# enac-drones/dronesim

Measured on AMD Instinct MI355X. Metric: drone-steps/sec (num_drones x env steps/s), higher is better.
Workload: dtype f32

## Files before the change

dronesim_amd/csrc/dsim_step.hip:

```cpp
#include "dsim_kernels.h"

template <bool NOISE, bool NT, bool EXT, bool CH = false, int SUB = 0, bool ACT = false, bool TC = false, bool MD = false>
__global__ __launch_bounds__(256, EXT ? 3 : DSIM_STEP_WAVES) void k_step_fast(StepK a) {
  static_assert(!MD || (SUB == 1 && !EXT && !ACT && !CH && TC), "MD: the plain single-sub-step TC instances");
  const DevType& T = a.types[0];
  const long long sfs = a.st.field_stride, tfs = a.tg.field_stride;
  const unsigned sl = 4u * kv_lane(a.st, threadIdx.x), tl = 4u * kv_lane(a.tg, threadIdx.x);
  const long long i0 = (long long)blockIdx.x * 256;
  float* const sb = a.st.base + kv_off(a.st, i0);
  const unsigned bt = a.tgt_tiles == ~0u ? (blockIdx.x & a.tgt_mask) : blockIdx.x % a.tgt_tiles;
  const long long i0t = (!EXT && !ACT) ? (long long)bt * 256 : i0;
  const float* const tb = a.tg.base + kv_off(a.tg, i0t);
  Rigid s;
  CtrlMem<4> m;
  Target tg;
  constexpr bool TAB = NOISE && (EXT || SUB != 1);
  __shared__ NoiseTab ntab_[TAB ? 1 : 0 + 1];
  const NoiseTab* const ntab = TAB ? &ntab_[0] : nullptr;
  if (TAB) noise_tab_init(ntab_[0], threadIdx.x);
  load_rigid<NT>(sb, sfs, sl, s);
  load_mem<4, NT, CH || MD>(sb, sfs, sl, m);
  if (TAB) __syncthreads();
  if (CH || MD) { m.last_vel = s.vel; m.last_rates = MD ? body_rates_apart(s.q, s.w) : body_rates(s.q, s.w); }
  const long long i = i0 + threadIdx.x;
  if (NOISE && a.step_index_dev) a.step_index += *a.step_index_dev;
  V3 pos_e;
  float yaw_e;
  if (!EXT) {
    load_target<NT, TC>(tb, tfs, tl, a.tc, tg);
    if (ACT) {
      float act[4];
#pragma unroll
      for (int j = 0; j < 4; ++j) act[j] = clampf(a.action[(long long)j * a.n_pad + i], T.pmin[j], T.pmax[j]);
      quad_substeps<NOISE ? 1 : 0, 4, false, SUB, false, -1, SUB == 0, TAB ? 1 : 0>(T, a, i, s, act, a.step_index, V3{-0.0f, -0.0f, -0.0f}, nullptr, -1, ntab);
    } else {
      quad_substeps<NOISE ? 1 : 0, 4, false, SUB, false, -1, SUB == 0, TAB ? 1 : 0>(T, a, i, s, m.cmd, a.step_index, V3{-0.0f, -0.0f, -0.0f}, nullptr, -1, ntab);
    }
    if (SUB == 1) ground_watch(T, s, a.fb.counters, i < a.n);
    indi_quad<false>(T, a.dt_ctrl, s, tg, m, pos_e, yaw_e);
  } else {
    int wp = 0;
    if (a.wp_table) wp = a.wp_counter[i]; else load_target<NT>(tb, tfs, tl, tg);
    for (int k = 0; k < a.n_steps; ++k) {
      if (a.wp_table) waypoint_target(a, i, wp, tg);
      if (a.substeps > 1) quad_substeps<NOISE ? 1 : 0, 4, false, 0, false, -1, true, TAB ? 1 : 0>(T, a, i, s, m.cmd, a.step_index + k, V3{-0.0f, -0.0f, -0.0f}, nullptr, -1, ntab);
      else quad_substeps<NOISE ? 1 : 0, 4, false, 0, false, -1, false, TAB ? 1 : 0>(T, a, i, s, m.cmd, a.step_index + k, V3{-0.0f, -0.0f, -0.0f}, nullptr, -1, ntab);
      ground_watch(T, s, a.fb.counters, i < a.n);
      indi_quad<false>(T, a.dt_ctrl, s, tg, m, pos_e, yaw_e);
      wp = waypoint_next(wp, a.n_wp);
    }
    if (a.wp_table) a.wp_counter[i] = wp;
  }
  const unsigned so = pin_lane_offset(sl);
  store_rigid<NT>(sb, sfs, so, s);
  store_mem<4, NT, CH>(sb, sfs, so, m);
  if (!EXT && SUB != 1) ground_watch(T, s, a.fb.counters, i < a.n);
}

template <bool NOISE, bool NT, bool S1, bool ACT = false, bool MD = false>
__global__ __launch_bounds__(256, (MD && !NOISE) ? 7 : DSIM_HEXA_WAVES) void k_step_hexa(StepK a) {
  static_assert(!MD || (S1 && !ACT), "MD: the single-sub-step instances without an explicit action");
  const DevType& T = a.types[0];
  const long long sfs = a.st.field_stride, tfs = a.tg.field_stride;
  const unsigned sl = 4u * kv_lane(a.st, threadIdx.x), tl = 4u * kv_lane(a.tg, threadIdx.x);
  const long long i0 = (long long)blockIdx.x * 256;
  float* const sb = a.st.base + kv_off(a.st, i0);
  const float* const tb = a.tg.base + kv_off(a.tg, i0);
  constexpr bool TAB = NOISE && !S1;
  __shared__ NoiseTab ntab_[TAB ? 1 : 0 + 1];
  const NoiseTab* const ntab = TAB ? &ntab_[0] : nullptr;
  if (TAB) noise_tab_init(ntab_[0], threadIdx.x);
  Rigid s;
  CtrlMem<6> m;
  Target tg;
  load_rigid<NT>(sb, sfs, sl, s);
  load_mem<6, NT, MD>(sb, sfs, sl, m);
  load_target<NT>(tb, tfs, tl, tg);
  if (MD) { m.last_vel = s.vel; m.last_rates = body_rates_apart(s.q, s.w); }
  if (TAB) __syncthreads();
  const long long i = i0 + threadIdx.x;
  if (NOISE && a.step_index_dev) a.step_index += *a.step_index_dev;
  V3 pos_e;
  float yaw_e;
  if (ACT) {
    float act[6];
#pragma unroll
    for (int j = 0; j < 6; ++j) act[j] = clampf(a.action[(long long)j * a.n_pad + i], T.pmin[j], T.pmax[j]);
    hexa_substeps<NOISE, false, S1, false, !S1, TAB ? 1 : 0>(T, a, i, s, act, a.step_index, V3{-0.0f, -0.0f, -0.0f}, -1, ntab);
  } else {
    hexa_substeps<NOISE, false, S1, false, !S1, TAB ? 1 : 0>(T, a, i, s, m.cmd, a.step_index, V3{-0.0f, -0.0f, -0.0f}, -1, ntab);
  }
  indi_hexa<false>(T, a.dt_ctrl, s, tg, m, pos_e, yaw_e, a.fb, i);
  float* const sb2 = (DSIM_LATE_STORE_BASE && (!S1 || DSIM_LATE_STORE_BASE_S1)) ? const_cast<float*>(opaque_after(sb, s.pos.x)) : sb;
  const unsigned so = pin_lane_offset(sl);
  store_rigid<NT>(sb2, sfs, so, s);
  store_mem<6, NT>(sb2, sfs, so, m);
  ground_watch(T, s, a.fb.counters, i < a.n);
}

struct MatK { KView st; long long n_pad; };
__global__ __launch_bounds__(256) void k_materialize(MatK a) {
  const long long i = (long long)blockIdx.x * 256 + threadIdx.x;
  if (i >= a.n_pad) return;
  float* p = a.st.base + kv_off(a.st, i);
  const long long fs = a.st.field_stride;
  Rigid s;
  load_rigid(p, fs, 0u, s);
  const V3 wb = body_rates(s.q, s.w);
  p[13 * fs] = s.vel.x; p[14 * fs] = s.vel.y; p[15 * fs] = s.vel.z;
  p[16 * fs] = wb.x; p[17 * fs] = wb.y; p[18 * fs] = wb.z;
}

template <int KIND, bool NOISE, bool NT, bool S1, bool ACT = false>
__device__ __forceinline__ void run_body(const StepK& a, long long i0, long long lo, long long last, int run_type,
                                         const NoiseTab* tab = nullptr) {
  constexpr bool HEXA = KIND != DSIM_DEV_KIND_QUAD;
  const long long i = i0 + threadIdx.x;
  if (i >= last || i < lo) return;
  const DevType& T = a.types[run_type];
  const long long sfs = a.st.field_stride, tfs = a.tg.field_stride;
  const unsigned sl = 4u * kv_lane(a.st, threadIdx.x), tl = 4u * kv_lane(a.tg, threadIdx.x);
  float* const sb = a.st.base + kv_off(a.st, i0);
  const float* const tb = a.tg.base + kv_off(a.tg, i0);
  constexpr int NA = HEXA ? 6 : 4;
  Rigid s;
  CtrlMem<NA> m;
  Target tg;
  load_rigid<NT>(sb, sfs, sl, s);
  load_mem<NA, NT>(sb, sfs, sl, m);
  load_target<NT>(tb, tfs, tl, tg);
  V3 ext = v3(0, 0, 0);
  if (a.ext_force) ext = v3(a.ext_force[i], a.ext_force[a.n_pad + i], a.ext_force[2 * a.n_pad + i]);
  unsigned long long step_index = a.step_index;
  if (NOISE && a.step_index_dev) step_index += *a.step_index_dev;
  V3 pos_e;
  float yaw_e;
  const long long nid = NOISE ? noise_id(a, i) : -1LL;
  float act[NA];
#pragma unroll
  for (int j = 0; j < NA; ++j) act[j] = ACT ? clampf(a.action[(long long)j * a.n_pad + i], T.pmin[j], T.pmax[j]) : m.cmd[j];
  if constexpr (HEXA) {
    hexa_substeps<NOISE, false, S1, false, !S1, (NOISE && !S1 && !ACT) ? 1 : 0>(T, a, i, s, act, step_index, ext, nid, tab);
    if constexpr (KIND == DSIM_DEV_KIND_HEXA) indi_hexa<false>(T, a.dt_ctrl, s, tg, m, pos_e, yaw_e, a.fb, i);
    else indi_quad<false, 6>(T, a.dt_ctrl, s, tg, m, pos_e, yaw_e);
  } else {
    quad_substeps<NOISE ? 1 : 0, 4, false, S1 ? 1 : 0, false, -1, !S1, (NOISE && !S1 && !ACT) ? 1 : 0>(T, a, i, s, act, step_index, ext, nullptr, nid, tab);
    indi_quad<false>(T, a.dt_ctrl, s, tg, m, pos_e, yaw_e);
  }
  const unsigned so = pin_lane_offset(sl);
  float* const sb2 = (DSIM_LATE_STORE_BASE && !S1) ? const_cast<float*>(opaque_after(sb, s.pos.x)) : sb;
  store_rigid<NT>(sb2, sfs, so, s);
  store_mem<NA, NT>(sb2, sfs, so, m);
  ground_watch(T, s, a.fb.counters, i < a.n);
  if (a.bin.count && i < a.n) bin_entry<KIND != DSIM_DEV_KIND_HEXA_QUADLAW>(a.bin, s.pos.x, s.pos.y, s.pos.z, a.bin.local_offset + i);
}
template <int KIND, bool NOISE, bool NT, bool S1>
__global__ __launch_bounds__(256, KIND ? DSIM_HEXA_WAVES : DSIM_STEP_WAVES) void k_step_run(StepK a) {
  DSIM_NOISE_TAB(NOISE && !S1, 256);
  run_body<KIND, NOISE, NT, S1>(a, a.first + (long long)blockIdx.x * 256, a.lo, a.last, a.run_type, ntab);
}
template <bool NOISE, bool NT, bool S1, bool ACT>
__global__ __launch_bounds__(256, 3) void k_step_runs(StepK a, RunTab rt) {
  DSIM_RUN_OF_BLOCK(rt, ro, blockIdx.x);
  DSIM_NOISE_TAB(NOISE && !S1 && !ACT, 256);
  if (ro.hexa) run_body<DSIM_DEV_KIND_HEXA, NOISE, NT, S1, ACT>(a, ro.i0, ro.lo, ro.last, ro.type, ntab);
  else run_body<DSIM_DEV_KIND_QUAD, NOISE, NT, S1, ACT>(a, ro.i0, ro.lo, ro.last, ro.type, ntab);
}

static int step_dyn(dsim_ctx* ctx, const dsim_step_args* args, const StepK& a, hipStream_t st_) {
  const int rc = dyn_check(ctx, args, a);
  if (rc) return rc;
  if (!a.tg.base) return DSIM_E_ARG;
  ctx->prebin.valid = false;
  return dyn_launch(true, a, stream_policy(args, a.n_pad, 256.0), st_);
}

static int step_runs(dsim_ctx* ctx, int64_t n, const dsim_step_args* args, const StepCall& c, StepK& a,
                     const dsim_type_run* runs, int n_runs, hipStream_t st_) {
  const dim3 b(256);
  const bool nt = stream_policy(args, a.n_pad, 240.0);
  bool any_hexa = false;
  bin_next_prepare(ctx, n, args, &a, st_);
  for (int r = 0; r < n_runs; ++r) {
    if (!run_valid(ctx, a.n_pad, runs[r])) return DSIM_E_ARG;
    any_hexa |= ctx->h_types[runs[r].type].kind == DSIM_KIND_HEXA6DOF;
  }
  if (any_hexa) {
    const int rc = fb_open_queue(ctx, &a, st_);
    if (rc) return rc;
  }
  const bool per_run_pays = a.substeps > 1 && a.n_pad >= (1LL << 20) && !args->action;
  const bool one_launch = !c.any_quadlaw6 && !per_run_pays;
  if (n_runs <= DSIM_MAX_TYPES && (n_runs >= 2 || args->action) && one_launch) {
    RunTab rt;
    const int blocks = make_runtab(ctx, a.n_pad, runs, n_runs, &rt, &any_hexa);
    if (blocks < 0) return blocks;
    if (blocks > 0) {
      const dim3 g((unsigned)blocks);
      with_flags([&](auto N, auto NT, auto S1, auto ACT) {
        hipLaunchKernelGGL((k_step_runs<N(), NT() && !ACT(), S1(), ACT()>), g, b, 0, st_, a, rt);
      }, c.noise, nt, a.substeps == 1, args->action != nullptr);
    }
  } else {
    for (int r = 0; r < n_runs; ++r) {
      const dsim_type_run& run = runs[r];
      if (run.count == 0) continue;
      a.first = run.first & ~255LL; a.lo = run.first; a.last = run.first + run.count; a.run_type = run.type;
      const dim3 g(grid_for(a.last - a.first));
      const int kind = ctx->h_types[run.type].kind;
      with_flags([&](auto N, auto NT, auto S1) {
        if (kind == DSIM_KIND_HEXA6DOF) hipLaunchKernelGGL((k_step_run<DSIM_DEV_KIND_HEXA, N(), NT(), S1()>), g, b, 0, st_, a);
        else if (kind == DSIM_KIND_HEXA_QUADLAW) hipLaunchKernelGGL((k_step_run<DSIM_DEV_KIND_HEXA_QUADLAW, N(), false, S1()>), g, b, 0, st_, a);
        else hipLaunchKernelGGL((k_step_run<DSIM_DEV_KIND_QUAD, N(), NT(), S1()>), g, b, 0, st_, a);
      }, c.noise, nt, a.substeps == 1);
    }
  }
  if (any_hexa) fb_finish(ctx, a, st_);
  bin_next_commit(ctx, n, args, a);
  return (int)hipGetLastError();
}

static long long step_quad_tiles(const dsim_step_args* args, const StepCall& c, const StepK& a, hipStream_t st_) {
  const bool nt = stream_policy(args, a.n_pad, 232.0);
  const long long tiles = a.n_pad / 256;
  if (tiles == 0) return 0;
  const dim3 g((unsigned)tiles), b(256);
  const bool ext = c.multi;
  const bool ch = (args->options & DSIM_OPT_CHAINED) != 0;
  const bool tc = tgt_const_honoured(args);
  const bool md = (args->options & DSIM_OPT_MEM_DERIVED) != 0;
  with_flags([&](auto N, auto NT, auto CH, auto S1, auto TC, auto MD) {
    if (ext) hipLaunchKernelGGL((k_step_fast<N(), NT(), true, CH()>), g, b, 0, st_, a);
    else if (args->action) hipLaunchKernelGGL((k_step_fast<N(), false, false, false, S1() ? 1 : 0, true>), g, b, 0, st_, a);
    else hipLaunchKernelGGL((k_step_fast<N(), NT(), false, CH(), S1() ? 1 : 0, false, TC(), MD() && S1() && !CH() && TC()>), g, b, 0, st_, a);
  }, c.noise, nt, ch, a.substeps == 1, tc, md);
  return tiles * 256;
}

static int step_hexa_tiles(dsim_ctx* ctx, const dsim_step_args* args, const StepCall& c, StepK& a, hipStream_t st_, long long* first) {
  const long long tiles = a.n_pad / 256;
  const bool nt = stream_policy(args, a.n_pad, 248.0);
  const int rc = fb_open_queue(ctx, &a, st_);
  if (rc) return rc;
  const dim3 g((unsigned)tiles), b(256);
  const bool md = (args->options & DSIM_OPT_MEM_DERIVED) != 0;
  with_flags([&](auto N, auto NT, auto S1, auto ACT, auto MD) {
    hipLaunchKernelGGL((k_step_hexa<N(), NT() && !ACT(), S1(), ACT(), MD() && S1() && !ACT()>), g, b, 0, st_, a);
  }, c.noise, nt, a.substeps == 1, args->action != nullptr, md);
  *first = tiles * 256;
  if (*first >= a.n_pad) fb_finish(ctx, a, st_);
  return DSIM_OK;
}

extern "C" {

int dsim_step(dsim_ctx* ctx, void* stream, int64_t n, dsim_view state, dsim_view targets,
              const dsim_step_args* args) {
  StepK a;
  int rc = fill_stepk(ctx, n, state, &targets, args, &a);
  if (rc) return rc;
  const StepCall c = classify_step(ctx, args, a);
  const hipStream_t st_ = (hipStream_t)stream;
  if (args->options & DSIM_OPT_DYN) return step_dyn(ctx, args, a, st_);
  if (args->options & DSIM_OPT_CALLER_IO) return DSIM_E_UNSUPPORTED;
  ctx->prebin.valid = false;
  if ((args->options & (DSIM_OPT_DRAG | DSIM_OPT_GROUND)) && c.six)
    return DSIM_E_UNSUPPORTED;
  if ((args->options & DSIM_OPT_CHAINED) && (!c.uni || c.six || args->action || c.replay || args->ext_force ||
                                             c.off_fast_path || !c.whole_tiles))
    return DSIM_E_UNSUPPORTED;
  const bool runs_ok = !c.replay && !c.multi && !c.off_fast_path && a.tg.base && !(args->options & DSIM_OPT_CHAINED);
  dsim_type_run whole;
  const bool whole_as_run = c.uni && runs_ok && (args->ext_force || (c.any_quadlaw6 && !args->action));
  const CallRuns cr = call_runs(args, a.n_pad, INT_MAX, whole_as_run, whole);
  if (cr.n_runs > 0 && runs_ok && (!args->action || (cr.n_runs <= DSIM_MAX_TYPES && !c.any_quadlaw6)))
    return step_runs(ctx, n, args, c, a, cr.runs, cr.n_runs, st_);
  long long first = 0;
  bool fb_open = false;
  if (c.uni && !c.six && !(args->action && c.multi) && !c.replay && !args->ext_force && !c.off_fast_path)
    first = step_quad_tiles(args, c, a, st_);
  if (c.uni && c.six && ctx->h_types[0].kind == DSIM_KIND_HEXA6DOF && !c.replay && !args->ext_force && !c.multi &&
      a.n_pad >= 256 && !c.off_fast_path) {
    rc = step_hexa_tiles(ctx, args, c, a, st_, &first);
    if (rc) return rc;
    fb_open = true;
  }
  if (first < a.n_pad) return step_general(ctx, n, state, targets, args, c, a, first, fb_open, st_);
  return (int)hipGetLastError();
}

int dsim_materialize(dsim_ctx* ctx, void* stream, int64_t n, dsim_view state) {
  if (!ctx || n <= 0 || n > state.n_pad) return DSIM_E_ARG;
  MatK a;
  int rc = make_kview(state, 20 + ctx->max_act, &a.st);
  if (rc) return rc;
  a.n_pad = state.n_pad;
  hipLaunchKernelGGL(k_materialize, dim3(grid_for(a.n_pad)), dim3(256), 0, (hipStream_t)stream, a);
  return (int)hipGetLastError();
}

}
```

Baseline: 34.81 billion.

## Add constant-target hexa kernel and memory-derived hints for mixed-run steps

Adds a specialised hexa step kernel that is used when targets are constant and there is one sub-step with no action. It loads targets through the constant-target path, derives the last velocity and rates from state instead of loading them when the memory-derived option is set, and uses higher occupancy launch bounds when noise is off. The mixed-run kernel gets a similar HINT mode that skips the memory fields and uses constant targets. The aim is to cut global memory traffic per drone, at the cost of more template instances and narrow preconditions that must hold for the results to stay correct.

```diff
diff --git a/dronesim_amd/csrc/dsim_step.hip b/dronesim_amd/csrc/dsim_step.hip
--- a/dronesim_amd/csrc/dsim_step.hip
+++ b/dronesim_amd/csrc/dsim_step.hip
@@ -98,6 +98,35 @@
   ground_watch(T, s, a.fb.counters, i < a.n);
 }
 
+template <bool NOISE, bool NT, bool MD>
+__global__ __launch_bounds__(256, !NOISE ? 7 : DSIM_HEXA_WAVES) void k_step_hexa_tc(StepK a) {
+  const DevType& T = a.types[0];
+  const long long sfs = a.st.field_stride, tfs = a.tg.field_stride;
+  const unsigned sl = 4u * kv_lane(a.st, threadIdx.x), tl = 4u * kv_lane(a.tg, threadIdx.x);
+  const long long i0 = (long long)blockIdx.x * 256;
+  float* const sb = a.st.base + kv_off(a.st, i0);
+  const unsigned bt = a.tgt_tiles == ~0u ? (blockIdx.x & a.tgt_mask) : blockIdx.x % a.tgt_tiles;
+  const float* const tb = a.tg.base + kv_off(a.tg, (long long)bt * 256);
+  Rigid s;
+  CtrlMem<6> m;
+  Target tg;
+  load_rigid<NT>(sb, sfs, sl, s);
+  load_mem<6, NT, MD>(sb, sfs, sl, m);
+  load_target<NT, true>(tb, tfs, tl, a.tc, tg);
+  if (MD) { m.last_vel = s.vel; m.last_rates = body_rates_apart(s.q, s.w); }
+  const long long i = i0 + threadIdx.x;
+  if (NOISE && a.step_index_dev) a.step_index += *a.step_index_dev;
+  V3 pos_e;
+  float yaw_e;
+  hexa_substeps<NOISE, false, true, false, false, 0>(T, a, i, s, m.cmd, a.step_index, V3{-0.0f, -0.0f, -0.0f}, -1, nullptr);
+  indi_hexa<false>(T, a.dt_ctrl, s, tg, m, pos_e, yaw_e, a.fb, i);
+  float* const sb2 = (DSIM_LATE_STORE_BASE && DSIM_LATE_STORE_BASE_S1) ? const_cast<float*>(opaque_after(sb, s.pos.x)) : sb;
+  const unsigned so = pin_lane_offset(sl);
+  store_rigid<NT>(sb2, sfs, so, s);
+  store_mem<6, NT>(sb2, sfs, so, m);
+  ground_watch(T, s, a.fb.counters, i < a.n);
+}
+
 struct MatK { KView st; long long n_pad; };
 __global__ __launch_bounds__(256) void k_materialize(MatK a) {
   const long long i = (long long)blockIdx.x * 256 + threadIdx.x;
@@ -111,7 +140,7 @@
   p[16 * fs] = wb.x; p[17 * fs] = wb.y; p[18 * fs] = wb.z;
 }
 
-template <int KIND, bool NOISE, bool NT, bool S1, bool ACT = false>
+template <int KIND, bool NOISE, bool NT, bool S1, bool ACT = false, bool HINT = false>
 __device__ __forceinline__ void run_body(const StepK& a, long long i0, long long lo, long long last, int run_type,
                                          const NoiseTab* tab = nullptr) {
   constexpr bool HEXA = KIND != DSIM_DEV_KIND_QUAD;
@@ -127,8 +156,9 @@
   CtrlMem<NA> m;
   Target tg;
   load_rigid<NT>(sb, sfs, sl, s);
-  load_mem<NA, NT>(sb, sfs, sl, m);
-  load_target<NT>(tb, tfs, tl, tg);
+  load_mem<NA, NT, HINT>(sb, sfs, sl, m);
+  load_target<NT, HINT>(tb, tfs, tl, a.tc, tg);
+  if (HINT) { m.last_vel = s.vel; m.last_rates = body_rates_apart(s.q, s.w); }
   V3 ext = v3(0, 0, 0);
   if (a.ext_force) ext = v3(a.ext_force[i], a.ext_force[a.n_pad + i], a.ext_force[2 * a.n_pad + i]);
   unsigned long long step_index = a.step_index;
@@ -159,12 +189,13 @@
   DSIM_NOISE_TAB(NOISE && !S1, 256);
   run_body<KIND, NOISE, NT, S1>(a, a.first + (long long)blockIdx.x * 256, a.lo, a.last, a.run_type, ntab);
 }
-template <bool NOISE, bool NT, bool S1, bool ACT>
+template <bool NOISE, bool NT, bool S1, bool ACT, bool HINT = false>
 __global__ __launch_bounds__(256, 3) void k_step_runs(StepK a, RunTab rt) {
+  static_assert(!HINT || (S1 && !ACT), "HINT: the single-sub-step instances without an explicit action");
   DSIM_RUN_OF_BLOCK(rt, ro, blockIdx.x);
   DSIM_NOISE_TAB(NOISE && !S1 && !ACT, 256);
-  if (ro.hexa) run_body<DSIM_DEV_KIND_HEXA, NOISE, NT, S1, ACT>(a, ro.i0, ro.lo, ro.last, ro.type, ntab);
-  else run_body<DSIM_DEV_KIND_QUAD, NOISE, NT, S1, ACT>(a, ro.i0, ro.lo, ro.last, ro.type, ntab);
+  if (ro.hexa) run_body<DSIM_DEV_KIND_HEXA, NOISE, NT, S1, ACT, HINT>(a, ro.i0, ro.lo, ro.last, ro.type, ntab);
+  else run_body<DSIM_DEV_KIND_QUAD, NOISE, NT, S1, ACT, HINT>(a, ro.i0, ro.lo, ro.last, ro.type, ntab);
 }
 
 static int step_dyn(dsim_ctx* ctx, const dsim_step_args* args, const StepK& a, hipStream_t st_) {
@@ -197,9 +228,10 @@
     if (blocks < 0) return blocks;
     if (blocks > 0) {
       const dim3 g((unsigned)blocks);
-      with_flags([&](auto N, auto NT, auto S1, auto ACT) {
-        hipLaunchKernelGGL((k_step_runs<N(), NT() && !ACT(), S1(), ACT()>), g, b, 0, st_, a, rt);
-      }, c.noise, nt, a.substeps == 1, args->action != nullptr);
+      const bool hint = (args->options & DSIM_OPT_MEM_DERIVED) && tgt_const_honoured(args) && !args->ext_force && !a.bin.count;
+      with_flags([&](auto N, auto NT, auto S1, auto ACT, auto H) {
+        hipLaunchKernelGGL((k_step_runs<N(), NT() && !ACT(), S1(), ACT(), H() && S1() && !ACT()>), g, b, 0, st_, a, rt);
+      }, c.noise, nt, a.substeps == 1, args->action != nullptr, hint);
     }
   } else {
     for (int r = 0; r < n_runs; ++r) {
@@ -244,9 +276,11 @@
   if (rc) return rc;
   const dim3 g((unsigned)tiles), b(256);
   const bool md = (args->options & DSIM_OPT_MEM_DERIVED) != 0;
-  with_flags([&](auto N, auto NT, auto S1, auto ACT, auto MD) {
-    hipLaunchKernelGGL((k_step_hexa<N(), NT() && !ACT(), S1(), ACT(), MD() && S1() && !ACT()>), g, b, 0, st_, a);
-  }, c.noise, nt, a.substeps == 1, args->action != nullptr, md);
+  const bool tc = tgt_const_honoured(args) && a.substeps == 1 && !args->action;
+  with_flags([&](auto N, auto NT, auto S1, auto ACT, auto MD, auto TC) {
+    if constexpr (TC()) hipLaunchKernelGGL((k_step_hexa_tc<N(), NT(), MD()>), g, b, 0, st_, a);
+    else hipLaunchKernelGGL((k_step_hexa<N(), NT() && !ACT(), S1(), ACT(), MD() && S1() && !ACT()>), g, b, 0, st_, a);
+  }, c.noise, nt, a.substeps == 1, args->action != nullptr, md, tc);
   *first = tiles * 256;
   if (*first >= a.n_pad) fb_finish(ctx, a, st_);
   return DSIM_OK;
```

Result: slower. 34.37 billion (-1.3%).
